# RandomMike1280/AlphaZero-Reversi

Measured on AMD Instinct MI355X. Metric: self-play board-steps/sec @ 800 sims/move, 8x8 Reversi, higher is better.
Workload: dtype u64 rules + f32 NN (fp32 as 2-part f16 split on MFMA)

## Files before the change

alphazero-reversi_amd/csrc/rvz_engine.hip:

```cpp
#include <hip/hip_bf16.h>
#include <hip/hip_runtime.h>
#include <math.h>
#include <stdint.h>
#include <stdio.h>
#include <stdlib.h>
#include <string.h>

#include <string>
#include <vector>

#include "../../include/rvz.h"
#include "rvz_h2.hip.h"
#include "rvz_pow.hip.h"
#include "rvz_rules.hip.h"
#include "rvz_trace.h"

using namespace rvz;

namespace {

constexpr int WAVE = 64;
constexpr int WPB = 4;
constexpr int PATH_CAP = 64;
constexpr int RNG_DRAWS = 64;
// ... 293 lines not shown
    if (copies == 0) return;
    const int path_reg = lane < plen ? v.path[g * PATH_CAP + lane] : 0;
    Node* nodes = v.nodes + (size_t)g * v.M;
    if (lane < plen) nodes[path_reg].n += copies;
    if (lane == 0) v.pend[g] = 0;
    __builtin_amdgcn_fence(__ATOMIC_SEQ_CST, "workgroup");
    if (v.stats) ab += 8ull + 4ull * plen + 8ull * plen;
}

template <int BS>
__device__ __forceinline__ int memo_expand_backup(const View& v, int g, int lane, int leaf,
                                                  uint32_t lm, int path_reg, int plen,
                                                  uint32_t lk, int copies,
                                                  unsigned long long& ab) {
    constexpr int NSQ = Geo<BS>::NSQ;
    Node* nodes = v.nodes + (size_t)g * v.M;
    uint32_t* meta = v.meta + (size_t)g * v.M;
    const int nch = link_nchild(lk), ob = 1 + link_block(lk) * NSQ;
    Node oc;
    uint32_t ocm = 0;
    if (lane < nch) {
        oc = nodes[ob + lane];
        ocm = meta[ob + lane];
    }
    const float val = v.bval[(size_t)g * 2 * v.E + link_block(lk)];
    const int e = v.nexp[g];
    const int base = 1 + e * NSQ;
    if (base + NSQ > v.M) {
        if (lane == 0) atomicOr(v.err, ERR_POOL);
        return -1;
    }
    float prior = lane < nch ? oc.p : 0.0f;
    if (leaf == 0 && v.noise_eps > 0.0f) {
        if (lane < nch) prior = root_noise_mix(v, g, m_sq(ocm), prior);
    }
    if (lane < nch) {
        Node c;
        c.n = 0; c.w = 0.0f; c.p = prior;
        const bool expd = m_nchild(ocm) > 0 && !m_term(ocm);
        c.c = __uint_as_float(expd ? link_pack(ob + lane, m_nchild(ocm), m_block(ocm))
                                   : LINK_NONE);
        nodes[base + lane] = c;
        meta[base + lane] = meta_pack(m_sq(ocm), 3 - m_turn(lm));
    }
    if (lane == 0) {
        meta[leaf] = lm | ((uint32_t)nch << 11) | ((uint32_t)e << 18);
        v.nexp[g] = e + 1;
        v.bval[(size_t)g * 2 * v.E + e] = val;
    }
    ab += 20ull * nch + 8 + 20ull * nch + 12 + 32ull * plen;
    return backup_path(nodes, path_reg, plen, val, copies, lane, true);
}

template <int BS, typename XT>
__device__ __forceinline__ int select_phase(const View& v, int g, int lane, int first, int bsz,
                                             int eb,
                                             const GameS& root, uint32_t root_meta, int root_n,
                                             uint32_t carry,
                                             XT* __restrict__ leaf_x, int32_t* __restrict__ need,
                                             unsigned long long& ab,
                                             uint64_t* leaf_bits = nullptr,
                                             bool unread = false) {
    constexpr int NSQ = Geo<BS>::NSQ;
    Node* nodes = v.nodes + (size_t)g * v.M;
    uint32_t* meta = v.meta + (size_t)g * v.M;
    if (first) {
        root_meta = meta_pack(0, root.side);
        root_n = 0;
        const int half = (v.memo && link_ok(carry) && (link_node(carry) - 1) / NSQ < v.E) ? 1 : 0;
        if (lane == 0) {
            Node r;
            r.n = 0; r.w = 0.0f; r.p = 1.0f; r.c = __int_as_float(0x7fc00000);
            nodes[0] = r;
            meta[0] = root_meta;
            v.nexp[g] = half * v.E;
        }
        const uint64_t rl = root.over ? 0ull : legal_wave<BS>(mine(root), theirs(root), lane);
        if (lane == 0) v.root_legal[g] = rl;
        if (v.noise_eps > 0.0f && rl != 0ull) root_noise_sample(v, g, lane, root, rl);
        ab += 20 + 8;
    }
    ab += 32 + 8;
    int copies = 0, plen = 0, path_reg = 0;
    if (!root.over) {
        int remaining = bsz;
        for (;;) {
            WALK_STAT(0, 1);
            WT_NOW(tw0);
            GameS sim = root;
            int depth = 0, node = 0, parent_n = root_n;
            uint32_t m = root_meta;
            uint32_t lk = first ? carry : LINK_NONE;
            path_reg = 0;
            int fp_ci = 0, fp_b = -1, fp_turn = 0;
            float fp_sb = 0.0f;
            bool truncated = false;
            int fp_sq = 0;
            for (;;) {
                const int nch = m_nchild(m);
                if (m_term(m) || nch == 0) break;
                const int base = 1 + m_block(m) * NSQ;
                Node c;
                uint32_t cm = 0;
                if (lane < nch) {
                    c = nodes[base + lane];
                    cm = meta[base + lane];
                } else {
                    c.n = 0; c.w = 0.0f; c.p = 0.0f; c.c = 0.0f;
                }
                float score = 0.0f;
                bool wrote = false;
                if (lane < nch) {
                    if (c.n == 0) {
                        score = INFINITY;
                    } else if (!isnan(c.c)) {
                        score = c.c;
                    } else {
                        const float sq_np = sqrt_count(parent_n);
                        score = ucb_score(c, sq_np, 3 - m_turn(m), v.cpuct);
                        nodes[base + lane].c = score;
                        wrote = true;
                    }
                }
                WALK_STAT(1, 1);
                const int ci = wave_argmax_first(score, lane < nch, lane);
                const int bsib = wave_argmax_first(score, lane < nch && lane != ci, lane);
                const float sbs = lane_bcast(score, bsib);
                const int turn_c = 3 - m_turn(m);
                if (v.stats) ab += 16ull * nch + 4ull * nch + 4ull * __popcll(__ballot(wrote));
                node = base + ci;
                m = (uint32_t)lane_bcast((int)cm, ci);
// ... 1405 lines not shown
    {
        double frac = e->gate_frac, us = e->gate_us, late = e->gate_late_us;
        if (frac < 0.0) {
            frac = RVZ_PLAY_GATE_FRAC;
            us = RVZ_PLAY_GATE_US;
            late = RVZ_PLAY_GATE_LATE_US;
        }
        if (const char* gs = getenv("RVZ_PLAY_GATE")) {
            double f = 0.0, u = 0.0, l = 0.0;
            const int n = sscanf(gs, "%lf,%lf,%lf", &f, &u, &l);
            frac = n >= 2 ? f : 0.0;
            us = u;
            late = n >= 3 ? l : 0.0;
        }
        pa.gate_frac = (queue && frac > 0.0 && us > 0.0)
                           ? (unsigned)(fmin(frac, 1.0) * 65536.0 + 0.5) : 0u;
        pa.gate_t = (unsigned)(us * 100.0);
        pa.gate_late = late > 0.0 ? (unsigned)(late * 100.0) : 0u;
    }
    sc += play_qwords(G);
    pa.x = sc;
    sc += play_al4(G * 3 * e->NSQ);
    pa.need = reinterpret_cast<int32_t*>(sc);
    sc += play_al4(G);
    pa.work = sc;
    sc += play_al4(G * 192);
    pa.logits = sc;
    sc += play_al4(G * e->NPOL);
    pa.value = sc;
    pa.ovf = a->ovf;
    pa.gpw = queue ? -a->games_per_workgroup : a->games_per_workgroup;
    pa.plies = a->plies;
    pa.skip_last = a->skip_last_eval && e->cfg.num_simulations > e->cfg.batch_size ? 1 : 0;
    pa.reset = a->reset ? 1 : 0;
    pa.S = e->cfg.num_simulations;
    pa.B = e->cfg.batch_size;
    pa.temperature = a->temperature;
    pa.seeds = a->seeds;
    pa.stride = a->seed_stride;
    pa.ply_ctr = a->plies_done;
    pa.done = a->games_done;
    pa.out_idx = a->out_idx;
    pa.out_p = a->out_p;
    pa.hist = a->hist;
    pa.rows = reinterpret_cast<unsigned long long*>(a->rows_evaluated);
    pa.budget = a->ply_budget;
    pa.tab = nullptr;
    pa.tclaim = nullptr;
    pa.tgen = nullptr;
    pa.tmask = 0;
    pa.tmaxd = 0;
    pa.tstats = reinterpret_cast<unsigned long long*>(a->table_stats);
    pa.unread = reinterpret_cast<unsigned long long*>(a->rows_unread);
    pa.rec_black = a->rec_black;
    pa.rec_white = a->rec_white;
    pa.rec_side = a->rec_side;
    pa.rec_p = a->rec_p;
    if ((a->rec_black || a->rec_white || a->rec_side || a->rec_p) &&
        !(a->rec_black && a->rec_white && a->rec_side && a->rec_p)) {
        e->err = "rvz_play: rec_black, rec_white, rec_side and rec_p go together";
        return RVZ_EINVAL;
    }
    if (e->tab) {
        if (e->tab_blob != a->blob) {
            if (e->tab_blob) {
                hipStreamCaptureStatus cs = hipStreamCaptureStatusNone;
                if (hipStreamIsCapturing(e->stream, &cs) == hipSuccess &&
                    cs != hipStreamCaptureStatusNone) {
                    e->err = "rvz_play: another weight blob than the table's while the stream is "
                             "capturing (play once eagerly with this evaluator before capturing)";
                    return RVZ_EINVAL;
                }
                const int r = table_bump(e);
                if (r != RVZ_OK) return r;
            }
            e->tab_blob = a->blob;
        }
        pa.tab = e->tab;
        pa.tclaim = e->tclaim;
        pa.tgen = e->tgen;
        pa.tmask = (unsigned)(e->tslots - 1);
        pa.tmaxd = e->tmaxd;
    }
    pa.spin_limit = 1u << 26;
    if (const char* sl = getenv("RVZ_PLAY_SPIN_LIMIT")) pa.spin_limit = (unsigned)strtoul(sl, nullptr, 10);
    e->searching = 0;
    if (e->BS == 8)
        return a->filters == 64    ? play_launch<64, 2, 2, 4, 8, 2>(e, v, pa, 2)
               : a->filters == 128 ? play_launch<128, 1, 2, 4, 8, 2>(e, v, pa, 2)
                                   : play_launch<256, 1, 4, 4, 8, 1>(e, v, pa, 1);
    return a->filters == 64 ? play_launch<64, 3, 2, 4, 6, 2>(e, v, pa, 2)
                            : play_launch<128, 1, 2, 3, 6, 2>(e, v, pa, 2);
}

struct rvz_timer {
    std::vector<hipEvent_t> ev;
};

int rvz_timer_create(int32_t n, rvz_timer** out) {
    if (n <= 0 || !out) return RVZ_EINVAL;
    rvz_timer* t = new rvz_timer;
    t->ev.resize(n, nullptr);
    for (auto& e : t->ev) {
        if (hipEventCreateWithFlags(&e, hipEventDisableSystemFence) != hipSuccess) {
            for (auto& f : t->ev)
                if (f) (void)hipEventDestroy(f);
// ... 106 lines not shown
```

alphazero-reversi_amd/csrc/rvz_play.hip.h:

```cpp

struct PlayArgs {
    const float* prm;
    Layout L;
    const uint16_t* blob;
    int n_blocks;
    float* x;
    int32_t* need;
    float* work;
    float* logits;
    float* value;
    float* ovf;
    int gpw, plies, skip_last, reset, S, B;
    double temperature;
    int64_t* seeds;
    int64_t stride;
    int64_t* ply_ctr;
    int64_t* done;
    int32_t* out_idx;
    double* out_p;
    int32_t* hist;
    unsigned long long* rows;
    const int32_t* budget;
    unsigned spin_limit;
    unsigned long long* tab;
    unsigned* tclaim;
    const unsigned* tgen;
    unsigned tmask;
    int tmaxd;
    unsigned long long* tstats;
    unsigned long long* unread;
    uint64_t* rec_black;
    uint64_t* rec_white;
    int32_t* rec_side;
    double* rec_p;
    unsigned* q_next;
    unsigned* q_done;
    int n_groups;
    unsigned long long* gate;
    unsigned gate_frac;
    unsigned gate_t;
    unsigned gate_late;
};
constexpr int PLAY_GPW_MAX = 64;
template <int F, int BS>
__host__ __device__ constexpr bool play_heads_lds() { return F == 64 && BS == 8; }
template <int F, int BS>
__host__ __device__ constexpr int play_gpw_max() {
    return play_heads_lds<F, BS>() ? 8 : PLAY_GPW_MAX;
}
enum : int { PF_QUEUED = 1, PF_READY = 2, PF_DONE = 4, PF_EVAL = 8, PF_HELD = 16 };
constexpr int32_t ERR_SCHED = 16;

template <int BS>
struct TabGeo {
    static constexpr int NSQ = Geo<BS>::NSQ;
    static constexpr int NG = NSQ + 8;
    static constexpr int STRIDE = (NG + 7) / 8 * 8;
};
constexpr int TAB_PROBES = 8;

__device__ __forceinline__ uint64_t tab_mix(uint64_t z) {
    z ^= z >> 30;
    z *= 0xbf58476d1ce4e5b9ull;
    z ^= z >> 27;
    z *= 0x94d049bb133111ebull;
    return z ^ (z >> 31);
}
__device__ __forceinline__ uint64_t tab_hash(uint64_t P, uint64_t O, uint64_t V) {
    return tab_mix(P ^ tab_mix(O ^ tab_mix(V + 0x9e3779b97f4a7c15ull)));
}
template <int NSQ>
__device__ __forceinline__ uint32_t tab_key_word(int idx, uint64_t P, uint64_t O, uint64_t V) {
    const int k = idx - (NSQ + 2);
    const uint64_t w = k < 2 ? P : (k < 4 ? O : V);
    return (k & 1) ? (uint32_t)(w >> 32) : (uint32_t)w;
}

template <int BS>
__device__ __forceinline__ int tab_read(const unsigned long long* __restrict__ tab, uint32_t sl,
                                         uint32_t gen, uint64_t P, uint64_t O, uint64_t V,
                                         int lane, uint64_t& x0, uint64_t& x1) {
    using T = TabGeo<BS>;
    constexpr int NSQ = T::NSQ, NG = T::NG;
    const unsigned long long* e = tab + (size_t)sl * T::STRIDE;
    x0 = 0;
    x1 = 0;
    if (lane < NG) x0 = __hip_atomic_load(e + lane, __ATOMIC_RELAXED, __HIP_MEMORY_SCOPE_AGENT);
    if (NG > 64 && lane < NG - 64)
        x1 = __hip_atomic_load(e + 64 + lane, __ATOMIC_RELAXED, __HIP_MEMORY_SCOPE_AGENT);
    bool stale = false, other = false;
    if (lane < NG) {
        stale |= (uint32_t)(x0 >> 32) != gen;
        if (lane >= NSQ + 2) other |= (uint32_t)x0 != tab_key_word<NSQ>(lane, P, O, V);
    }
// ... 145 lines not shown
    asm volatile("" : "+s"(p));
    return *(const PlayCtx*)p;
}

#ifdef RVZ_PLAY_TIMING
__device__ unsigned long long g_play_t[16384][12];
#define PT_NOW(t) const unsigned long long t = __builtin_amdgcn_s_memtime()
#define PT_ADD(i, v) if (tid == 0 && blockIdx.x < 16384) g_play_t[blockIdx.x][i] += (v)
#else
#define PT_NOW(t)
#define PT_ADD(i, v)
#endif

template <int F, int NBOARD, int CTW, int PTW, int BS, int OCC>
__global__ __launch_bounds__(256) __attribute__((amdgpu_waves_per_eu(OCC, OCC)))
void k_play(PlayCtx ctx0) {
    (void)ctx0;
    using WT = WaveTilesH<F, CTW, PTW>;
    constexpr bool ILV = RVZ_H2_ILV && NBOARD == 2 && BS == 8 && PTW == 4 && WT::CG == 2;
    using GH = GeoH<NBOARD, BS, 64 * CTW * H2_TM / F, ILV>;
    using C = CfgH<F, GH::NPIX>;
    constexpr int NPOL = Geo<BS>::NPOL;
    constexpr bool HLDS = play_heads_lds<F, BS>();
    constexpr int GMAX = play_gpw_max<F, BS>();
    constexpr int HROW = heads_in_floats(BS) / 16;
    constexpr int SP_BYTES = WPB * (NPOL + 7) * 8;
    static_assert(heads_in_floats(BS) * 4 <= C::RMAX, "heads rows fit");
    static_assert(SP_BYTES + WPB * 624 * 4 <= C::RMAX, "act / reset scratch fits");
    __shared__ __attribute__((aligned(16))) char smem[C::BYTES];
    __shared__ int st_k[GMAX];
    __shared__ int st_f[GMAX];
    __shared__ int st_p[GMAX];
    __shared__ uint64_t st_bits[GMAX * 3];
    __shared__ uint64_t q_bits[(GMAX + NBOARD) * 3];
    __shared__ __attribute__((aligned(16))) float hin[HLDS ? GMAX * HROW : 4];
    __shared__ int q_rows[GMAX + 16];
    __shared__ int s_nq;
    __shared__ float vpart[4][16];
    __shared__ int s_task[2];
    __shared__ unsigned s_tgen;
    const int tid = threadIdx.x;
    const int wave = __builtin_amdgcn_readfirstlane(tid >> 6);
    int E, G, gpw, total, queue, task_plies;
    {
        const PlayCtx& c = play_ctx();
        E = c.v.E;
        G = c.v.G;
        gpw = c.a.gpw;
        queue = c.a.q_next != nullptr;
        total = queue ? c.a.n_groups * c.a.plies : 0;
        task_plies = queue ? 1 : c.a.plies;
    }
    bool ovf = false;
    __shared__ unsigned s_cnt[4];
    if (tid < 4) s_cnt[tid] = 0u;
    if (tid == 0) {
        const PlayArgs& a = play_ctx().a;
        s_tgen = a.tab ? __hip_atomic_load(a.tgen, __ATOMIC_RELAXED, __HIP_MEMORY_SCOPE_AGENT) : 0u;
    }
    double* sp = reinterpret_cast<double*>(smem) + wave * (NPOL + 7);
    uint32_t* key = reinterpret_cast<uint32_t*>(smem + SP_BYTES) + wave * 624;
    if constexpr (F >= 128 && BS == 8) {
        const PlayArgs& a = play_ctx().a;
        if (tid == 0 && a.gate_frac > 0) gate_running(a.gate, 1);
    }
    PT_NOW(t_start);
    for (int task_i = 0;; ++task_i) {
        int gi, ply0;
        if (!queue) {
            if (task_i > 0) break;
            gi = blockIdx.x;
            ply0 = 0;
        } else {
            PT_NOW(t_q0);
            if (tid == 0) {
                const PlayCtx& c = play_ctx();
                const PlayArgs& a = c.a;
                const bool failed = __hip_atomic_load(c.v.err, __ATOMIC_RELAXED,
                                                      __HIP_MEMORY_SCOPE_AGENT) & ERR_SCHED;
                const unsigned t =
                    failed ? (unsigned)total
                           : __hip_atomic_fetch_add(a.q_next, 1u, __ATOMIC_RELAXED,
                                                    __HIP_MEMORY_SCOPE_AGENT);
                int tg = -1, tp = 0;
                if ((int)t < total) {
                    tg = (int)(t % (unsigned)a.n_groups);
                    tp = (int)(t / (unsigned)a.n_groups);
                    unsigned spins = 0;
                    while ((int)__hip_atomic_load(a.q_done + tg, __ATOMIC_RELAXED,
                                                  __HIP_MEMORY_SCOPE_AGENT) < tp) {
                        __builtin_amdgcn_s_sleep(4);
                        ++spins;
                        if (spins > a.spin_limit ||
                            ((spins & 1023u) == 0 &&
                             (__hip_atomic_load(c.v.err, __ATOMIC_RELAXED,
                                                __HIP_MEMORY_SCOPE_AGENT) & ERR_SCHED))) {
                            atomicOr(c.v.err, ERR_SCHED);
                            tg = -1;
                            break;
                        }
                    }
                    __builtin_amdgcn_fence(__ATOMIC_ACQUIRE, "agent");
                    asm volatile("s_waitcnt vmcnt(0)" ::: "memory");
                }
                s_task[0] = tg;
                s_task[1] = tp;
            }
            __syncthreads();
// ... 3 lines not shown
            PT_NOW(t_q1);
            PT_ADD(8, t_q1 - t_q0);
            PT_ADD(9, 1);
        }
        const int g0 = gi * gpw;
        const int ng = min(gpw, G - g0);
        {
            const int32_t* bud = play_ctx().a.budget;
            for (int j = tid; j < ng; j += 256) {
                st_k[j] = 0;
                st_f[j] = (bud && ply0 >= bud[g0 + j]) ? PF_DONE : 0;
                st_p[j] = 0;
            }
        }
        __syncthreads();
        for (;;) {
            PT_NOW(t_c0);
            for (int j = wave; j < ng; j += WPB) {
                const PlayCtx& c = play_ctx();
                const View& v = c.v;
                const PlayArgs& a = c.a;
                const int lane = opaque_tid() & 63;
                const int g = g0 + j;
                int f = __builtin_amdgcn_readfirstlane(st_f[j]);
                if (f & (PF_QUEUED | PF_DONE)) continue;
                int k = __builtin_amdgcn_readfirstlane(st_k[j]);
                int np = __builtin_amdgcn_readfirstlane(st_p[j]);
                WT_NOW(ft_step);
                FT_CNT();
                for (;;) {
                    unsigned long long ab = 0;
                    if (k < E) {
                        const int first = k == 0;
                        const GameS root = load_game(v, g);
                        uint32_t root_meta = 0, carry = LINK_NONE;
                        int root_n = 0;
                        if (!first) {
                            root_meta = v.meta[(size_t)g * v.M];
                            root_n = v.nodes[(size_t)g * v.M].n;
                        } else if (v.memo) {
                            carry = v.carry[g];
                        }
                        if (f & PF_READY) {
                            WT_NOW(ft_e);
                            const ExpIn x = expand_load<BS>(v, g, lane, a.logits, a.value);
                            const int rn =
                                expand_backup_phase<BS>(v, g, lane, x, 1, &root_meta, ab);
                            if (rn >= 0) root_n = rn;
                            f &= ~PF_READY;
                            FT_ADD(0, ft_e);
                        }
                        const int bsz = min(a.B, a.S - k * a.B);
                        const bool unread = a.skip_last && !first && m_nchild(root_meta) >= E - 1;
                        const int copies = select_phase<BS, float>(v, g, lane, first, bsz, k, root,
                                                                   root_meta, root_n, carry, a.x,
                                                                   a.need, ab, st_bits + 3 * j,
                                                                   unread);
                        ++k;
                        if (copies < 0 && k < E && lane == 0) atomicAdd(&s_cnt[3], 1u);
                        if (copies > 0 && !(k == E && a.skip_last)) {
                            if (a.tab) {
                                const uint64_t P = st_bits[3 * j], O = st_bits[3 * j + 1],
                                               Vb = st_bits[3 * j + 2];
                                WT_NOW(ft_t);
                                const bool hit = __popcll(P | O) <= a.tmaxd &&
                                                 tab_lookup<BS>(a, s_tgen, P, O, Vb, lane, g);
                                WT_ADD(0, ft_t);
                                if (hit) {
                                    __builtin_amdgcn_fence(__ATOMIC_SEQ_CST, "workgroup");
                                    f |= PF_READY;
                                    if (lane == 0) atomicAdd(&s_cnt[1], 1u);
                                    continue;
                                }
                            }
                            f |= PF_QUEUED;
                            break;
                        }
                        continue;
                    }
                    WT_NOW(ft_a);
                    bool over = false;
                    double* outp = a.out_p;
                    if (a.rec_black) {
                        const size_t ri = (size_t)(ply0 + np) * v.G + g;
                        if (lane == 0) {
                            a.rec_black[ri] = v.black[g];
                            a.rec_white[ri] = v.white[g];
                            a.rec_side[ri] = v.status[(size_t)g * 4];
                        }
                        outp = a.rec_p + (size_t)(ply0 + np) * v.G * Geo<BS>::NPOL;
                    }
                    const int idx = act_game<BS>(v, g, lane, sp, (f & PF_READY) ? 1 : 2,
                                                 a.logits, 1, a.value, a.temperature, nullptr, 1,
                                                 a.out_idx, outp, &over);
                    f &= ~PF_READY;
                    int64_t sd = 0;
                    if (lane == 0) {
                        if (idx >= 0) a.ply_ctr[g] += 1;
                        if (a.hist) a.hist[(size_t)(ply0 + np) * v.G + g] = idx;
                        if (a.reset && over) {
                            a.done[g] += 1;
                            sd = a.seeds[g] + a.stride;
                            a.seeds[g] = sd;
                        }
                    }
                    if (a.reset && over) {
                        sd = __shfl(sd, 0);
                        reset_game<BS>(v, g, lane, (uint32_t)(sd & 0xFFFFFFFFll), key);
                    }
                    FT_ADD(1, ft_a);
// ... 94 lines not shown
                    const PlayArgs& a = play_ctx().a;
                    const uint64_t P = q_bits[3 * i], O = q_bits[3 * i + 1], Vb = q_bits[3 * i + 2];
                    if (__popcll(P | O) <= a.tmaxd)
                        if (tab_insert<BS>(a, s_tgen, P, O, Vb, opaque_tid() & 63, q_rows[i]) &&
                            (opaque_tid() & 63) == 0)
                            atomicAdd(&s_cnt[2], 1u);
                }
            }
            for (int j = tid; j < ng; j += 256)
                if (st_f[j] & PF_EVAL) st_f[j] = (st_f[j] & ~(PF_QUEUED | PF_EVAL)) | PF_READY;
            __syncthreads();
            PT_NOW(t_c4);
            PT_ADD(2, t_c4 - t_c3);
        }
        if (queue) {
            asm volatile("s_waitcnt vmcnt(0)" ::: "memory");
            __syncthreads();
            if (tid == 0) {
                __builtin_amdgcn_fence(__ATOMIC_RELEASE, "agent");
                asm volatile("s_waitcnt vmcnt(0)" ::: "memory");
                __hip_atomic_store(play_ctx().a.q_done + gi, (unsigned)(ply0 + 1), __ATOMIC_RELAXED,
                                   __HIP_MEMORY_SCOPE_AGENT);
            }
        }
    }
    if constexpr (F >= 128 && BS == 8) {
        const PlayArgs& a = play_ctx().a;
        if (tid == 0 && a.gate_frac > 0) gate_running(a.gate, -1);
    }
#ifdef RVZ_PLAY_TIMING
    {
        PT_NOW(t_end);
        PT_ADD(3, t_end - t_start);
        if (tid == 0 && blockIdx.x < 16384)
            g_play_t[blockIdx.x][10] = __builtin_amdgcn_s_memrealtime();
        if (tid == 0 && blockIdx.x < 16384)
            g_play_t[blockIdx.x][7] =
                ((unsigned long long)__builtin_amdgcn_s_getreg((31 << 11) | 20) << 32) |
                __builtin_amdgcn_s_getreg((31 << 11) | 4);
    }
#endif
    float* ovw = play_ctx().a.ovf;
    if (ovf && ovw) *ovw = 1.0f;
    unsigned long long* rows = play_ctx().a.rows;
    __syncthreads();
    if (rows && tid == 0) atomicAdd(rows, (unsigned long long)s_cnt[0]);
    unsigned long long* ts = play_ctx().a.tstats;
    if (ts && tid == 0) {
        if (s_cnt[1]) atomicAdd(ts, (unsigned long long)s_cnt[1]);
        if (s_cnt[2]) atomicAdd(ts + 1, (unsigned long long)s_cnt[2]);
    }
    unsigned long long* un = play_ctx().a.unread;
    if (un && tid == 0 && s_cnt[3]) atomicAdd(un, (unsigned long long)s_cnt[3]);
}
```

alphazero-reversi_amd/rvz/_lib.py:

```python
from __future__ import annotations

import ctypes as C
import math
import numbers
import os

import torch

_HERE = os.path.dirname(os.path.abspath(__file__))
LIB_PATH = os.environ.get("RVZ_LIB", os.path.join(_HERE, "librvz.so"))

RVZ_OK, RVZ_DONE = 0, 1
RVZ_LEAF_F32, RVZ_LEAF_BF16 = 0, 1
RVZ_DRAWS = 64
RVZ_SOLVE_MAX_EMPTIES = 14
RVZ_SOLVE_NOT_A_MOVE, RVZ_SOLVE_ABANDONED = -128, -127


class RvzError(RuntimeError):
    pass


class Config(C.Structure):
    _fields_ = [("board_size", C.c_int32), ("n_games", C.c_int32),
# ... 42 lines not shown
    "rvz_search_rows_total": (C.c_int, [_P, C.POINTER(C.c_int64)]),
    "rvz_timer_create": (C.c_int, [C.c_int32, C.POINTER(C.c_void_p)]),
    "rvz_timer_record": (C.c_int, [_P, C.c_int32, _P]),
    "rvz_timer_elapsed": (C.c_int, [_P, C.c_int32, C.c_int32, C.POINTER(C.c_float)]),
    "rvz_timer_destroy": (None, [_P]),
    "rvz_search_skip": (C.c_int, [_P]),
    "rvz_search_visits": (C.c_int, [_P, _P]),
    "rvz_act": (C.c_int, [_P, C.c_double, _P, C.c_int32, _P, _P]),
    "rvz_act_schedule": (C.c_int, [_P, C.c_int32, C.c_double]),
    "rvz_action_probs": (C.c_int, [C.c_int32, C.c_int32, _P, _P, _P, _P, _P, _P, _P]),
    "rvz_solve": (C.c_int, [C.c_int32, C.c_int32, _P, _P, _P, C.c_int32, C.c_int64, _P, _P, _P,
                            _P]),
    "rvz_solve_window": (C.c_int, [C.c_int32, C.c_int32, _P, _P, _P, C.c_int32, C.c_int64,
                                   C.c_int32, C.c_int32, C.c_int32, _P, _P, _P, _P]),
    "rvz_solve_moves": (C.c_int, [C.c_int32, C.c_int32, _P, _P, _P, C.c_int32, C.c_int64,
                                  C.c_int32, C.c_int32, C.c_int32, _P, _P, _P, _P]),
    "rvz_play_scratch_size": (C.c_int64, [_P]),
    "rvz_play": (C.c_int, [_P, _P]),
    "rvz_play_table": (C.c_int, [_P, C.c_int64, C.c_int32]),
    "rvz_play_gate": (C.c_int, [_P, C.c_double, C.c_double, C.c_double]),
    "rvz_counters": (C.c_int, [_P, C.POINTER(C.c_int64)]),
    "rvz_stats_enable": (C.c_int, [_P, C.c_int32]),
    "rvz_stats_read": (C.c_int, [_P, C.POINTER(C.c_int64)]),
    "rvz_timing_enable": (C.c_int, [_P, C.c_int32]),
    "rvz_timing_read": (C.c_int, [_P, C.POINTER(C.c_double), C.POINTER(C.c_int32)]),
    "rvz_tree_nodes": (C.c_int, [_P]),
    "rvz_tree_export": (C.c_int, [_P, _P, _P]),
    "rvz_footprint": (C.c_int, [_P, C.POINTER(C.c_int64), C.POINTER(C.c_int64)]),
    "rvz_resnet_params_size": (C.c_int64, [C.c_int32, C.c_int32, C.c_int32]),
    "rvz_resnet_work_size": (C.c_int64, [C.c_int32]),
    "rvz_resnet_heads_fc": (C.c_int, [C.c_int32, _P, C.c_int32, _P, C.c_int32, C.c_int32, _P, _P,
                                      _P]),
    "rvz_resnet_h2_size": (C.c_int64, [C.c_int32, C.c_int32]),
    "rvz_resnet_h2_weights": (C.c_int, [_P, C.c_int32, C.c_int32, _P, _P]),
    "rvz_resnet_trunk_h2": (C.c_int, [C.c_int32, _P, C.c_int32, _P, _P, C.c_int32, C.c_int32,
                                      _P, _P]),
    "rvz_resnet_fwd_h2": (C.c_int, [C.c_int32, _P, C.c_int32, _P, _P, C.c_int32, C.c_int32, _P,
                                    _P, _P, _P]),
}

_lib = None


class PlayArgs(C.Structure):
    _fields_ = [("params", C.c_void_p), ("blob", C.c_void_p), ("filters", C.c_int32),
                ("blocks", C.c_int32), ("scratch", C.c_void_p), ("ovf", C.c_void_p),
                ("plies", C.c_int32), ("skip_last_eval", C.c_int32), ("reset", C.c_int32),
                ("games_per_workgroup", C.c_int32), ("temperature", C.c_double),
                ("seeds", C.c_void_p), ("seed_stride", C.c_int64), ("plies_done", C.c_void_p),
                ("games_done", C.c_void_p), ("out_idx", C.c_void_p), ("out_p", C.c_void_p),
                ("hist", C.c_void_p), ("rows_evaluated", C.c_void_p),
                ("ply_budget", C.c_void_p), ("table_stats", C.c_void_p),
                ("rec_black", C.c_void_p), ("rec_white", C.c_void_p), ("rec_side", C.c_void_p),
                ("rec_p", C.c_void_p), ("rows_unread", C.c_void_p)]


def load() -> C.CDLL:
    global _lib
    if _lib is None:
        if not os.path.exists(LIB_PATH):
            raise RvzError(f"{LIB_PATH} is missing: build it with `make -C alphazero-reversi_amd` "
                           "(there is no CPU fallback for the rvz hot path)")
        lib = C.CDLL(LIB_PATH, mode=C.RTLD_GLOBAL)
        for name, (res, args) in SIGNATURES.items():
            fn = getattr(lib, name)
            fn.restype = res
            fn.argtypes = args
        _lib = lib
    return _lib


_NO_EPSILON = object()


def check_noise_args(alpha, epsilon=_NO_EPSILON) -> None:
    try:
        a = float(alpha)
    except (TypeError, ValueError, OverflowError):
        raise RvzError(f"root noise: alpha must be a positive finite number, not {alpha!r}")
    if not 1.0e-37 <= a <= 3.0e38:
        raise RvzError(f"root noise: alpha must be positive and finite (float32), not {alpha!r}")
    if epsilon is not _NO_EPSILON:
        try:
            e = float(epsilon)
        except (TypeError, ValueError):
            raise RvzError(f"root noise: epsilon must be a number in [0, 1], not {epsilon!r}")
        if not 0.0 <= e <= 1.0:
            raise RvzError(f"root noise: epsilon must be in [0, 1], not {epsilon!r}")


def check_schedule_args(moves, late_temperature=0.0):
    if moves is None:
        return None
    if isinstance(moves, bool) or not isinstance(moves, numbers.Integral) or moves < 0:
        raise RvzError(f"temperature schedule: moves must be None or an int >= 0, not {moves!r}")
    if int(moves) > 2 ** 31 - 5:
        raise RvzError(f"temperature schedule: moves = {moves!r} is out of range")
    try:
        late = float(late_temperature)
    except (TypeError, ValueError, OverflowError):
        raise RvzError("temperature schedule: late_temperature must be a finite number >= 0, "
                       f"not {late_temperature!r}")
    if isinstance(late_temperature, bool) or not (0.0 <= late < math.inf):
        raise RvzError("temperature schedule: late_temperature must be a finite number >= 0, "
                       f"not {late_temperature!r}")
    return int(moves), late

# ... 54 lines not shown
```

alphazero-reversi_amd/rvz/engine.py:

```python
from __future__ import annotations

import ctypes as C
from typing import Callable, Optional, Sequence, Tuple

import torch

from . import _lib
from ._lib import RVZ_DONE, RVZ_LEAF_BF16, RVZ_LEAF_F32, RvzError, check, ptr

U64 = 0xFFFFFFFFFFFFFFFF
SOLVE_MAX_EMPTIES = _lib.RVZ_SOLVE_MAX_EMPTIES
SOLVE_NOT_A_MOVE = _lib.RVZ_SOLVE_NOT_A_MOVE
SOLVE_ABANDONED = _lib.RVZ_SOLVE_ABANDONED


def to_signed64(x: int) -> int:
    x &= U64
    return x - (1 << 64) if x >> 63 else x


def to_unsigned64(x: int) -> int:
    return int(x) & U64


# ... 162 lines not shown
        torch.cuda.current_stream(self.device).synchronize()

    def _env_snapshot(self):
        self._stream()
        b = torch.empty(self.n_games, dtype=torch.int64, device=self.device)
        w = torch.empty_like(b)
        st = torch.empty(self.n_games, 4, dtype=torch.int32, device=self.device)
        self._call("rvz_env_get", ptr(b), ptr(w), ptr(st))
        return b, w, st

    def solve(self, max_empties: int = SOLVE_MAX_EMPTIES, node_limit: int = 2 ** 24):
        b, w, st = self._env_snapshot()
        return solve(b, w, st, self.board_size, max_empties, node_limit)

    def solve_wld(self, max_empties: int = SOLVE_MAX_EMPTIES, node_limit: int = 2 ** 24,
                  order_min_empties: Optional[int] = None):
        b, w, st = self._env_snapshot()
        if order_min_empties is None:
            order_min_empties = WLD_ORDER_MIN_EMPTIES
        return solve_wld(b, w, st, self.board_size, max_empties, node_limit, order_min_empties)

    def solve_moves(self, max_empties: int = SOLVE_MAX_EMPTIES, node_limit: int = 2 ** 24,
                    alpha: int = -64, beta: int = 64, order_min_empties: int = 0):
        b, w, st = self._env_snapshot()
        return solve_moves(b, w, st, self.board_size, max_empties, node_limit, alpha, beta,
                           order_min_empties)

    def solve_moves_wld(self, max_empties: int = SOLVE_MAX_EMPTIES, node_limit: int = 2 ** 24,
                        order_min_empties: Optional[int] = None):
        b, w, st = self._env_snapshot()
        if order_min_empties is None:
            order_min_empties = WLD_ORDER_MIN_EMPTIES
        return solve_moves_wld(b, w, st, self.board_size, max_empties, node_limit,
                               order_min_empties)

    def legal(self) -> torch.Tensor:
        self._stream()
        out = torch.empty(self.n_games, dtype=torch.int64, device=self.device)
        self._call("rvz_env_legal", ptr(out))
        return out

    def apply(self, sq: torch.Tensor) -> torch.Tensor:
        self._stream()
        s = sq.to(self.device, torch.int32).contiguous()
        ok = torch.empty(self.n_games, dtype=torch.int32, device=self.device)
        self._call("rvz_env_apply", ptr(s), ptr(ok))
        return ok

    def play_buffers(self, evaluator=None):
        if getattr(self, "play_rows", None) is None:
            self.play_rows = torch.zeros(1, dtype=torch.int64, device=self.device)
            self.table_stats = torch.zeros(2, dtype=torch.int64, device=self.device)
            self.play_unread = torch.zeros(1, dtype=torch.int64, device=self.device)
        n = self.lib.rvz_play_scratch_size(self._h)
        sc = getattr(self, "_play_scratch", None)
        if sc is None or sc.numel() < n:
            self._play_scratch = torch.zeros(n, dtype=torch.float32, device=self.device)
        if evaluator is not None and hasattr(evaluator, "ovf_word"):
            evaluator.ovf_word()

    def play(self, evaluator, plies: int, temperature: float, seeds: torch.Tensor, stride: int,
             plies_done: torch.Tensor, games_done: torch.Tensor, reset: bool = True,
             skip_last_eval: bool = False, hist: Optional[torch.Tensor] = None,
             games_per_workgroup: int = 0, budget: Optional[torch.Tensor] = None,
             records=None):
        from .network import LeafEvaluator
        if not isinstance(evaluator, LeafEvaluator):
            raise RvzError("play() runs the h2 LeafEvaluator inside the launch; another "
                           "evaluator goes through search() / act()")
        if evaluator.board_size != self.board_size or evaluator.device != self.device:
            raise RvzError("play(): the evaluator's board size / device differ from the engine's")
        for t, dt in ((seeds, torch.int64), (plies_done, torch.int64), (games_done, torch.int64)):
            if t.dtype != dt or t.numel() != self.n_games or not t.is_contiguous():
                raise RvzError("play: seeds / plies_done / games_done int64 [n_games]")
        if hist is not None and (hist.dtype != torch.int32 or hist.shape != (plies, self.n_games)
                                 or not hist.is_contiguous()):
            raise RvzError("play: hist int32 [plies, n_games]")
        if budget is not None and (budget.dtype != torch.int32 or budget.numel() != self.n_games
                                   or not budget.is_contiguous()
                                   or budget.device != self.device):
            raise RvzError("play: budget int32 [n_games] on the engine's device")
        rec = (None,) * 4
        if records is not None and hist is None:
            raise RvzError("play: records need hist (the moves of the recorded plies)")
        if records is not None:
            rb, rw, rs, rp = records
            G = self.n_games
            if not (rb.dtype == rw.dtype == torch.int64 and rs.dtype == torch.int32
                    and rp.dtype == torch.float64 and rb.shape == rw.shape == rs.shape
                    == (plies, G) and rp.shape == (plies, G, self.npol)
                    and all(t.is_contiguous() and t.device == self.device
                            for t in (rb, rw, rs, rp))):
                raise RvzError("play: records = (black int64, white int64 [plies, G], side int32 "
                               "[plies, G], p float64 [plies, G, npol]) on the engine's device")
            rec = tuple(t.data_ptr() for t in records)
        n = self.lib.rvz_play_scratch_size(self._h)
        ready = (getattr(self, "play_rows", None) is not None and
                 getattr(self, "_play_scratch", None) is not None and
                 self._play_scratch.numel() >= n and getattr(evaluator, "_ovf", None) is not None)
        if not ready:
            if torch.cuda.is_current_stream_capturing():
                raise RvzError("play() inside a graph capture before its buffers exist: call "
                               "Engine.play_buffers(evaluator) (or one eager play) first")
            self.play_buffers(evaluator)
        sc = self._play_scratch
        self._bind(evaluator)
        a = _lib.PlayArgs(evaluator.params.data_ptr(), evaluator.wsplit.data_ptr(),
                          evaluator.filters, evaluator.n_blocks, sc.data_ptr(),
                          evaluator.ovf_word().data_ptr(), int(plies), int(bool(skip_last_eval)),
                          int(bool(reset)), int(games_per_workgroup), float(temperature),
                          seeds.data_ptr(), int(stride), plies_done.data_ptr(),
                          games_done.data_ptr(), self.idx_buf.data_ptr(), self.p_buf.data_ptr(),
                          hist.data_ptr() if hist is not None else None,
                          self.play_rows.data_ptr(),
                          budget.data_ptr() if budget is not None else None,
                          self.table_stats.data_ptr(), *rec, self.play_unread.data_ptr())
        self._stream()
        self._call("rvz_play", C.byref(a))

    def _bind(self, evaluator):
        evs = self.__dict__.setdefault("_evaluators", [])
        if not any(e is evaluator for e in evs):
            evs.append(evaluator)
            reg = getattr(evaluator, "bind_engine", None)
            if reg is not None:
                reg(self)

    def table(self, slots: int = 1 << 20, max_discs: int = 14):
        self._stream()
        self._call("rvz_play_table", int(slots), int(max_discs))
        self.table_slots = int(slots)

    def play_gate(self, fraction: float = -1.0, timeout_us: float = 0.0, late_us: float = 0.0):
        self._call("rvz_play_gate", float(fraction), float(timeout_us), float(late_us))

    def root_noise(self, alpha: float, epsilon: float, salt: int = 0):
        _lib.check_noise_args(alpha, epsilon)
        self._call("rvz_search_root_noise", float(alpha), float(epsilon), int(salt) & 0xFFFFFFFF)
        self.noise = (float(alpha), float(epsilon), int(salt) & 0xFFFFFFFF)

    def temperature_schedule(self, moves: Optional[int], late_temperature: float = 0.0):
        sched = _lib.check_schedule_args(moves, late_temperature)
        if sched is None:
            self._call("rvz_act_schedule", 0, 0.0)
        else:
            self._call("rvz_act_schedule", 4 + sched[0], sched[1])
        self.schedule = sched

    def search_begin(self):
        self._call("rvz_search_begin")

    def search_step(self) -> bool:
        self._stream()
        rc = self._call("rvz_search_step", ptr(self.leaf_x), ptr(self.need))
        return rc != RVZ_DONE

    def compact(self, on: bool = True):
        self._call("rvz_search_compact", int(bool(on)))
        self.compact_leaves = bool(on)

    def memo(self, on: bool = True):
        self._stream()
        self._call("rvz_search_memo", int(bool(on)))
        self.memo_on = bool(on)

    def memo_reset(self):
        self._stream()
        self._call("rvz_search_memo_reset")

# ... 232 lines not shown
```

alphazero-reversi_amd/rvz/selfplay.py:

```python
from __future__ import annotations

import os
import time
from datetime import datetime
from typing import Callable, Dict, List, Optional, Sequence

import numpy as np
import torch

from .engine import Engine, board_canonical


class SelfPlayRunner:
    def __init__(self, engine: Engine, evaluator: Callable, temperature: float = 1.0,
                 fused_softmax: bool = True, autoreset: bool = False, seed_base: int = 42,
                 record: bool = False, max_plies: int = 60, seed_stride: int = None,
                 skip_last_eval: bool = False, fused_bookkeeping: bool = True,
                 fused: bool = False, temperature_schedule=None):
        self.eng = engine
        if temperature_schedule is not None:
            engine.temperature_schedule(*temperature_schedule)
        self.skip_last_eval = bool(skip_last_eval)
        self.fused = bool(fused)
        self.play_group = 0
        if self.fused and not fused_softmax:
            raise ValueError("the fused runner plays with fused_softmax")
        if self.fused and record and autoreset:
            raise ValueError("a recording fused runner plays whole games (no autoreset)")
        self.fused_bookkeeping = bool(fused_bookkeeping)
        self.evaluator = evaluator
        self.temperature = float(temperature)
        self.fused_softmax = fused_softmax
        self.autoreset = autoreset
        self.seed_base = seed_base
        self.seed_stride = engine.n_games if seed_stride is None else int(seed_stride)
        self.record = record
        G, dev = engine.n_games, engine.device
        self.seeds = (torch.arange(G, dtype=torch.int64, device=dev) + seed_base)
        self._plies = torch.zeros(G, dtype=torch.int64, device=dev)
        self._done = torch.zeros(G, dtype=torch.int64, device=dev)
        self.pre_black = torch.zeros(G, dtype=torch.int64, device=dev)
        self.pre_white = torch.zeros(G, dtype=torch.int64, device=dev)
        self.pre_status = torch.zeros(G, 4, dtype=torch.int32, device=dev)
        self.post_status = torch.zeros(G, 4, dtype=torch.int32, device=dev)
        self._seed32 = torch.zeros(G, dtype=torch.int32, device=dev)
        self._mask = torch.zeros(G, dtype=torch.uint8, device=dev)
        self.graph: Optional[torch.cuda.CUDAGraph] = None
        if record:
            self.rec_black = torch.zeros(max_plies, G, dtype=torch.int64, device=dev)
            self.rec_white = torch.zeros(max_plies, G, dtype=torch.int64, device=dev)
            self.rec_side = torch.zeros(max_plies, G, dtype=torch.int32, device=dev)
            self.rec_idx = torch.full((max_plies, G), -2, dtype=torch.int32, device=dev)
            self.rec_p = torch.zeros(max_plies, G, engine.npol, dtype=torch.float64, device=dev)
            self.rec_over = torch.zeros(max_plies, G, 4, dtype=torch.int32, device=dev)
        self.ply_index = 0
        if self.fused:
            engine.play_buffers(evaluator)

    @property
    def steps(self) -> torch.Tensor:
        return self._plies.sum()

    @property
    def games_done(self) -> torch.Tensor:
        return self._done.sum()

    def start(self):
        self.eng.reset(self.seeds)
        self.ply_index = 0

    def check(self):
        self.eng.check()

    def _body(self, plies: int = 1):
        eng = self.eng
        if self.fused:
            rec, hist = None, None
            if self.record:
                k, n = self.ply_index, plies
                if k + n > self.rec_idx.shape[0]:
                    raise ValueError("records are full (max_plies)")
                rec = (self.rec_black[k:k + n], self.rec_white[k:k + n], self.rec_side[k:k + n],
                       self.rec_p[k:k + n])
                hist = self.rec_idx[k:k + n]
            eng.play(self.evaluator, plies, self.temperature, self.seeds, self.seed_stride,
                     self._plies, self._done, reset=self.autoreset,
                     skip_last_eval=self.skip_last_eval, hist=hist,
                     games_per_workgroup=self.play_group, records=rec)
            if self.record:
                self.post_status.copy_(eng.get_state()[2])
            return
        if self.record:
            b, w, st = eng.get_state()
            self.pre_black.copy_(b)
            self.pre_white.copy_(w)
            self.pre_status.copy_(st)
        eng.search(self.evaluator, fused_softmax=self.fused_softmax,
                   skip_last_eval=self.skip_last_eval)
        idx, _ = eng.act(self.temperature, apply=True)
        if self.record:
            self.post_status.copy_(eng.get_state()[2])
        if self.fused_bookkeeping:
            eng.autoreset(idx, self.seeds, self.seed_stride, self._plies, self._done,
                          reset=self.autoreset)
            return
        self._plies += (idx >= 0).to(torch.int64)
        if self.autoreset:
            self.restart_finished(eng.get_state()[2])

    def restart_finished(self, status: torch.Tensor):
        over = status[:, 1]
        self._done += over.to(torch.int64)
        self.seeds += over.to(torch.int64) * self.seed_stride
        self._mask.copy_(over.to(torch.uint8))
        self._seed32.copy_(self.seeds.bitwise_and(0xFFFFFFFF).to(torch.int32))
        self.eng.reset_device(self._seed32, self._mask)

    def capture(self, plies: int = 1):
        if plies < 1 or (plies > 1 and self.record and not self.fused) or (self.record and
                                                                          self.fused):
            raise ValueError("plies >= 1; a recording runner captures one ply per graph (the "
                             "fused recording runner writes to the ply's record slice: use "
                             "play_record)")
        torch.cuda.synchronize(self.eng.device)
        g = torch.cuda.CUDAGraph()
        with torch.cuda.graph(g):
            if self.fused:
                self._body(plies)
            else:
                for _ in range(plies):
                    self._body()
        self.graph = g
        self.plies_per_call = int(plies)
        torch.cuda.synchronize(self.eng.device)

    plies_per_call = 1

    def play_record(self, plies: int):
        if not (self.fused and self.record):
            raise ValueError("play_record is the fused recording runner's")
        self._body(plies)
# ... 319 lines not shown
```

include/rvz.h:

```cpp
#ifndef RVZ_H
#define RVZ_H
#include <stdint.h>

#ifdef __cplusplus
extern "C" {
#endif

#define RVZ_OK 0
#define RVZ_DONE 1
#define RVZ_EINVAL (-22)
#define RVZ_ENOMEM (-12)
#define RVZ_EHIP (-5)
#define RVZ_EDEVICE (-71)

#define RVZ_LEAF_F32 0
#define RVZ_LEAF_BF16 1

#define RVZ_LIVE_STRIPE 128
#define RVZ_LIVE_PITCH 16

typedef struct rvz_engine rvz_engine;

typedef struct rvz_config {
    int32_t board_size;
// ... 48 lines not shown
                        const uint32_t *seed32, const int32_t *tag, uint32_t salt, double alpha,
                        float *out, uint32_t *out_bits, void *hip_stream);
int rvz_search_rows_total(rvz_engine *e, int64_t *out );
int rvz_search_visits(rvz_engine *e, int32_t *out);
int rvz_act(rvz_engine *e, double temperature, const double *u, int32_t apply, int32_t *out_idx,
            double *out_p);
int rvz_act_schedule(rvz_engine *e, int32_t from_discs, double late_temperature);
int rvz_action_probs(int32_t board_size, int32_t n, const int32_t *visits,
                     const double *temperature, const double *u, int32_t *out_idx, double *out_p,
                     int32_t *out_drew, void *hip_stream);

#define RVZ_SOLVE_MAX_EMPTIES 14
int rvz_solve(int32_t board_size, int32_t n, const uint64_t *black, const uint64_t *white,
              const int32_t *status, int32_t max_empties, int64_t node_limit, int32_t *out_score,
              int32_t *out_move, int64_t *out_nodes, void *hip_stream);
int rvz_solve_window(int32_t board_size, int32_t n, const uint64_t *black, const uint64_t *white,
                     const int32_t *status, int32_t max_empties, int64_t node_limit,
                     int32_t alpha, int32_t beta, int32_t order_min_empties,
                     int32_t *out_score, int32_t *out_move, int64_t *out_nodes, void *hip_stream);
#define RVZ_SOLVE_NOT_A_MOVE (-128)
#define RVZ_SOLVE_ABANDONED (-127)
int rvz_solve_moves(int32_t board_size, int32_t n, const uint64_t *black, const uint64_t *white,
                    const int32_t *status, int32_t max_empties, int64_t node_limit,
                    int32_t alpha, int32_t beta, int32_t order_min_empties, int32_t *out_scores,
                    int32_t *out_count, int64_t *out_nodes, void *hip_stream);

typedef struct rvz_play_args {
    const float *params;
    const uint16_t *blob;
    int32_t filters;
    int32_t blocks;
    float *scratch;
    float *ovf;
    int32_t plies;
    int32_t skip_last_eval;
    int32_t reset;
    int32_t games_per_workgroup;
    double temperature;
    int64_t *seeds;
    int64_t seed_stride;
    int64_t *plies_done;
    int64_t *games_done;
    int32_t *out_idx;
    double *out_p;
    int32_t *hist;
    int64_t *rows_evaluated;
    const int32_t *ply_budget;
    int64_t *table_stats;
    uint64_t *rec_black;
    uint64_t *rec_white;
    int32_t *rec_side;
    double *rec_p;
    int64_t *rows_unread;
} rvz_play_args;
int64_t rvz_play_scratch_size(const rvz_engine *e);
int rvz_play(rvz_engine *e, const rvz_play_args *a);
int rvz_play_table(rvz_engine *e, int64_t slots, int32_t max_discs);
int rvz_play_gate(rvz_engine *e, double fraction, double timeout_us, double late_us);

typedef struct rvz_timer rvz_timer;
int rvz_timer_create(int32_t n_events, rvz_timer **out);
int rvz_timer_record(rvz_timer *t, int32_t i, void *hip_stream);
int rvz_timer_elapsed(rvz_timer *t, int32_t i, int32_t j, float *ms );
void rvz_timer_destroy(rvz_timer *t);

int rvz_counters(const rvz_engine *e, int64_t *out2 );
int rvz_stats_enable(rvz_engine *e, int32_t on);
int rvz_stats_read(rvz_engine *e, int64_t *out3 );
int rvz_timing_enable(rvz_engine *e, int32_t on);
int rvz_timing_read(rvz_engine *e, double *out_ms , int32_t *out_n );
int rvz_tree_nodes(const rvz_engine *e);
int rvz_tree_export(rvz_engine *e, void *nodes_out, uint32_t *meta_out);
int rvz_footprint(const rvz_engine *e, int64_t *bytes_tree, int64_t *bytes_env);

int64_t rvz_resnet_params_size(int32_t board, int32_t filters, int32_t blocks);
int64_t rvz_resnet_work_size(int32_t n);
int rvz_resnet_heads_fc(int32_t board, const float *work, int32_t n, const float *params,
                        int32_t filters, int32_t blocks, float *logits, float *value,
                        void *hip_stream);

int64_t rvz_resnet_h2_size(int32_t filters, int32_t blocks);
int rvz_resnet_h2_weights(const float *params, int32_t filters, int32_t blocks, uint16_t *blob,
                          void *hip_stream);
int rvz_resnet_fwd_h2(int32_t board, const float *x, int32_t n, const float *params,
                      const uint16_t *blob, int32_t filters, int32_t blocks, float *work,
                      float *logits, float *value, void *hip_stream);
int rvz_resnet_trunk_h2(int32_t board, const float *x, int32_t n, const float *params,
                        const uint16_t *blob, int32_t filters, int32_t blocks, float *work,
                        void *hip_stream);
int32_t rvz_resnet_h2_grid(int32_t board, int32_t filters, int32_t n);
int rvz_resnet_fwd_h2_ex(int32_t board, const float *x, int32_t n, const float *params,
                         const uint16_t *blob, int32_t filters, int32_t blocks, float *work,
                         float *logits, float *value, const int32_t *n_live, void *hip_stream);
int rvz_resnet_trunk_h2_ex(int32_t board, const float *x, int32_t n, const float *params,
                           const uint16_t *blob, int32_t filters, int32_t blocks, float *work,
                           const int32_t *n_live, uint64_t *stamps, const uint32_t *stamp_ctr,
                           int32_t ring, void *hip_stream);
int rvz_resnet_heads_fc_ex(int32_t board, const float *work, int32_t n, const float *params,
                           int32_t filters, int32_t blocks, float *logits, float *value,
                           const int32_t *n_live, uint32_t *stamp_ctr, void *hip_stream);

#ifdef __cplusplus
}
#endif
#endif
```

Measured before the change: 1.666 million.

## Short-circuit root search when legal moves cover all batches

When a fresh root has at least E-1 legal moves and skip_last_eval is on, a new forced_search routine builds the root's children directly. It gives them deterministic visit counts, reuses subtrees linked from the previous move, and returns early, skipping the per-batch select/evaluate loop. The point is to avoid NN leaf evaluations and tree walks whose outcome the batch schedule already fixes. Risks: it assumes the search would spread visits across distinct children, and it writes zero priors with unevaluated children. It is enabled by default only for fused play with skip_last_eval and at least 3 batches, and adds a roots_unread counter.

Result: faster. 1.711 million, median of 6 (+2.7%).

```diff
diff --git a/alphazero-reversi_amd/csrc/rvz_engine.hip b/alphazero-reversi_amd/csrc/rvz_engine.hip
--- a/alphazero-reversi_amd/csrc/rvz_engine.hip
+++ b/alphazero-reversi_amd/csrc/rvz_engine.hip
@@ -369,6 +369,81 @@
     return backup_path(nodes, path_reg, plen, val, copies, lane, true);
 }
 
+struct Forced {
+    int E, S, B;
+};
+
+template <int BS>
+__device__ __noinline__ int forced_search(const View& v, int g, int lane, int side,
+                                          uint32_t root_meta, uint64_t rl, int half,
+                                          uint32_t carry, Forced fz) {
+    constexpr int NSQ = Geo<BS>::NSQ;
+    Node* nodes = v.nodes + (size_t)g * v.M;
+    uint32_t* meta = v.meta + (size_t)g * v.M;
+    const int L = __popcll(rl), nv = fz.E - 1;
+    const int e0 = half * v.E, base = 1 + e0 * NSQ;
+    const bool linked_root = v.memo && link_ok(carry);
+    const bool mine = lane < NSQ && ((rl >> lane) & 1ull);
+    const int idx = __popcll(rl & ((1ull << lane) - 1ull));
+    if (base + NSQ > v.M) {
+        if (lane == 0) atomicOr(v.err, ERR_POOL);
+        return 0;
+    }
+    uint32_t lk = LINK_NONE;
+    if (linked_root && mine) {
+        const int oc = 1 + link_block(carry) * NSQ + idx;
+        const uint32_t ocm = meta[oc];
+        if (m_nchild(ocm) > 0 && !m_term(ocm)) lk = link_pack(oc, m_nchild(ocm), m_block(ocm));
+    }
+    const bool visited = mine && idx < nv;
+    uint64_t lmask = __ballot(visited && link_ok(lk));
+    if (1 + (e0 + 1 + __popcll(lmask)) * NSQ > v.M) {
+        if (lane == 0) atomicOr(v.err, ERR_POOL);
+        lmask = 0ull;
+    }
+    const bool expd = (lmask >> lane) & 1ull;
+    const int ce = e0 + 1 + __popcll(lmask & ((1ull << lane) - 1ull));
+    if (mine) {
+        Node c;
+        c.n = visited ? min(fz.B, fz.S - (idx + 1) * fz.B) : 0;
+        c.w = 0.0f; c.p = 0.0f; c.c = __uint_as_float(LINK_NONE);
+        nodes[base + idx] = c;
+        uint32_t cm = meta_pack(lane, 3 - side);
+        if (expd) cm |= ((uint32_t)link_nchild(lk) << 11) | ((uint32_t)ce << 18);
+        meta[base + idx] = cm;
+    }
+    int e = e0 + 1;
+    for (uint64_t rest = lmask; rest != 0ull; rest &= rest - 1ull, ++e) {
+        const int s = __ffsll((unsigned long long)rest) - 1;
+        const uint32_t l = (uint32_t)__builtin_amdgcn_readlane((int)lk, s);
+        const int nch = link_nchild(l), ob = 1 + link_block(l) * NSQ, nb = 1 + e * NSQ;
+        if (lane < nch) {
+            const Node oc = nodes[ob + lane];
+            const uint32_t ocm = meta[ob + lane];
+            Node c;
+            c.n = 0; c.w = 0.0f; c.p = oc.p;
+            c.c = __uint_as_float(m_nchild(ocm) > 0 && !m_term(ocm)
+                                      ? link_pack(ob + lane, m_nchild(ocm), m_block(ocm))
+                                      : LINK_NONE);
+            nodes[nb + lane] = c;
+            meta[nb + lane] = meta_pack(m_sq(ocm), side);
+        }
+        if (lane == 0)
+            v.bval[(size_t)g * 2 * v.E + e] = v.bval[(size_t)g * 2 * v.E + link_block(l)];
+    }
+    if (lane == 0) {
+        Node r;
+        r.n = fz.S; r.w = 0.0f; r.p = 1.0f; r.c = __int_as_float(0x7fc00000);
+        nodes[0] = r;
+        meta[0] = root_meta | ((uint32_t)L << 11) | ((uint32_t)e0 << 18);
+        v.nexp[g] = e;
+        v.pend[g] = 0;
+        v.plen[g] = 0;
+    }
+    __builtin_amdgcn_fence(__ATOMIC_SEQ_CST, "workgroup");
+    return __popcll(__ballot(mine && idx < nv - 1 && !link_ok(lk))) + (linked_root ? 0 : 256);
+}
+
 template <int BS, typename XT>
 __device__ __forceinline__ int select_phase(const View& v, int g, int lane, int first, int bsz,
                                              int eb,
@@ -377,7 +452,7 @@
                                              XT* __restrict__ leaf_x, int32_t* __restrict__ need,
                                              unsigned long long& ab,
                                              uint64_t* leaf_bits = nullptr,
-                                             bool unread = false) {
+                                             bool unread = false, Forced fz = Forced{0, 0, 0}) {
     constexpr int NSQ = Geo<BS>::NSQ;
     Node* nodes = v.nodes + (size_t)g * v.M;
     uint32_t* meta = v.meta + (size_t)g * v.M;
@@ -394,6 +469,8 @@
         }
         const uint64_t rl = root.over ? 0ull : legal_wave<BS>(mine(root), theirs(root), lane);
         if (lane == 0) v.root_legal[g] = rl;
+        if (fz.E > 0 && !root.over && __popcll(rl) >= fz.E - 1)
+            return -2 - forced_search<BS>(v, g, lane, root.side, root_meta, rl, half, carry, fz);
         if (v.noise_eps > 0.0f && rl != 0ull) root_noise_sample(v, g, lane, root, rl);
         ab += 20 + 8;
     }
@@ -1905,6 +1982,8 @@
     pa.tmaxd = 0;
     pa.tstats = reinterpret_cast<unsigned long long*>(a->table_stats);
     pa.unread = reinterpret_cast<unsigned long long*>(a->rows_unread);
+    pa.skip_forced = a->skip_forced_roots && pa.skip_last ? 1 : 0;
+    pa.roots_unread = reinterpret_cast<unsigned long long*>(a->roots_unread);
     pa.rec_black = a->rec_black;
     pa.rec_white = a->rec_white;
     pa.rec_side = a->rec_side;
diff --git a/alphazero-reversi_amd/csrc/rvz_play.hip.h b/alphazero-reversi_amd/csrc/rvz_play.hip.h
--- a/alphazero-reversi_amd/csrc/rvz_play.hip.h
+++ b/alphazero-reversi_amd/csrc/rvz_play.hip.h
@@ -40,6 +40,8 @@
     unsigned gate_frac;
     unsigned gate_t;
     unsigned gate_late;
+    int skip_forced;
+    unsigned long long* roots_unread;
 };
 constexpr int PLAY_GPW_MAX = 64;
 template <int F, int BS>
@@ -291,8 +293,8 @@
         task_plies = queue ? 1 : c.a.plies;
     }
     bool ovf = false;
-    __shared__ unsigned s_cnt[4];
-    if (tid < 4) s_cnt[tid] = 0u;
+    __shared__ unsigned s_cnt[5];
+    if (tid < 5) s_cnt[tid] = 0u;
     if (tid == 0) {
         const PlayArgs& a = play_ctx().a;
         s_tgen = a.tab ? __hip_atomic_load(a.tgen, __ATOMIC_RELAXED, __HIP_MEMORY_SCOPE_AGENT) : 0u;
@@ -402,10 +404,20 @@
                         }
                         const int bsz = min(a.B, a.S - k * a.B);
                         const bool unread = a.skip_last && !first && m_nchild(root_meta) >= E - 1;
+                        const Forced fz{first && a.skip_forced ? E : 0, a.S, a.B};
                         const int copies = select_phase<BS, float>(v, g, lane, first, bsz, k, root,
                                                                    root_meta, root_n, carry, a.x,
                                                                    a.need, ab, st_bits + 3 * j,
-                                                                   unread);
+                                                                   unread, fz);
+                        if (copies <= -2) {
+                            k = E;
+                            const int left = -2 - copies;
+                            if (lane == 0) {
+                                if (left & 255) atomicAdd(&s_cnt[3], (unsigned)(left & 255));
+                                if (left >> 8) atomicAdd(&s_cnt[4], 1u);
+                            }
+                            continue;
+                        }
                         ++k;
                         if (copies < 0 && k < E && lane == 0) atomicAdd(&s_cnt[3], 1u);
                         if (copies > 0 && !(k == E && a.skip_last)) {
@@ -606,4 +618,6 @@
     }
     unsigned long long* un = play_ctx().a.unread;
     if (un && tid == 0 && s_cnt[3]) atomicAdd(un, (unsigned long long)s_cnt[3]);
-}
+    unsigned long long* ur = play_ctx().a.roots_unread;
+    if (ur && tid == 0 && s_cnt[4]) atomicAdd(ur, (unsigned long long)s_cnt[4]);
+}
diff --git a/alphazero-reversi_amd/rvz/_lib.py b/alphazero-reversi_amd/rvz/_lib.py
--- a/alphazero-reversi_amd/rvz/_lib.py
+++ b/alphazero-reversi_amd/rvz/_lib.py
@@ -118,7 +118,8 @@
                 ("hist", C.c_void_p), ("rows_evaluated", C.c_void_p),
                 ("ply_budget", C.c_void_p), ("table_stats", C.c_void_p),
                 ("rec_black", C.c_void_p), ("rec_white", C.c_void_p), ("rec_side", C.c_void_p),
-                ("rec_p", C.c_void_p), ("rows_unread", C.c_void_p)]
+                ("rec_p", C.c_void_p), ("rows_unread", C.c_void_p),
+                ("skip_forced_roots", C.c_int32), ("roots_unread", C.c_void_p)]
 
 
 def load() -> C.CDLL:
diff --git a/alphazero-reversi_amd/rvz/engine.py b/alphazero-reversi_amd/rvz/engine.py
--- a/alphazero-reversi_amd/rvz/engine.py
+++ b/alphazero-reversi_amd/rvz/engine.py
@@ -238,6 +238,8 @@
             self.play_rows = torch.zeros(1, dtype=torch.int64, device=self.device)
             self.table_stats = torch.zeros(2, dtype=torch.int64, device=self.device)
             self.play_unread = torch.zeros(1, dtype=torch.int64, device=self.device)
+        if getattr(self, "play_roots_unread", None) is None:
+            self.play_roots_unread = torch.zeros(1, dtype=torch.int64, device=self.device)
         n = self.lib.rvz_play_scratch_size(self._h)
         sc = getattr(self, "_play_scratch", None)
         if sc is None or sc.numel() < n:
@@ -249,7 +251,7 @@
              plies_done: torch.Tensor, games_done: torch.Tensor, reset: bool = True,
              skip_last_eval: bool = False, hist: Optional[torch.Tensor] = None,
              games_per_workgroup: int = 0, budget: Optional[torch.Tensor] = None,
-             records=None):
+             records=None, skip_forced_roots: bool = False):
         from .network import LeafEvaluator
         if not isinstance(evaluator, LeafEvaluator):
             raise RvzError("play() runs the h2 LeafEvaluator inside the launch; another "
@@ -282,6 +284,7 @@
             rec = tuple(t.data_ptr() for t in records)
         n = self.lib.rvz_play_scratch_size(self._h)
         ready = (getattr(self, "play_rows", None) is not None and
+                 getattr(self, "play_roots_unread", None) is not None and
                  getattr(self, "_play_scratch", None) is not None and
                  self._play_scratch.numel() >= n and getattr(evaluator, "_ovf", None) is not None)
         if not ready:
@@ -300,7 +303,8 @@
                           hist.data_ptr() if hist is not None else None,
                           self.play_rows.data_ptr(),
                           budget.data_ptr() if budget is not None else None,
-                          self.table_stats.data_ptr(), *rec, self.play_unread.data_ptr())
+                          self.table_stats.data_ptr(), *rec, self.play_unread.data_ptr(),
+                          int(bool(skip_forced_roots)), self.play_roots_unread.data_ptr())
         self._stream()
         self._call("rvz_play", C.byref(a))
 
diff --git a/alphazero-reversi_amd/rvz/selfplay.py b/alphazero-reversi_amd/rvz/selfplay.py
--- a/alphazero-reversi_amd/rvz/selfplay.py
+++ b/alphazero-reversi_amd/rvz/selfplay.py
@@ -16,11 +16,13 @@
                  fused_softmax: bool = True, autoreset: bool = False, seed_base: int = 42,
                  record: bool = False, max_plies: int = 60, seed_stride: int = None,
                  skip_last_eval: bool = False, fused_bookkeeping: bool = True,
-                 fused: bool = False, temperature_schedule=None):
+                 fused: bool = False, temperature_schedule=None, skip_forced_roots=None):
         self.eng = engine
         if temperature_schedule is not None:
             engine.temperature_schedule(*temperature_schedule)
         self.skip_last_eval = bool(skip_last_eval)
+        self.skip_forced_roots = (bool(fused) and bool(skip_last_eval) and engine.n_batches >= 3
+                                  if skip_forced_roots is None else bool(skip_forced_roots))
         self.fused = bool(fused)
         self.play_group = 0
         if self.fused and not fused_softmax:
@@ -86,7 +88,8 @@
             eng.play(self.evaluator, plies, self.temperature, self.seeds, self.seed_stride,
                      self._plies, self._done, reset=self.autoreset,
                      skip_last_eval=self.skip_last_eval, hist=hist,
-                     games_per_workgroup=self.play_group, records=rec)
+                     games_per_workgroup=self.play_group, records=rec,
+                     skip_forced_roots=self.skip_forced_roots)
             if self.record:
                 self.post_status.copy_(eng.get_state()[2])
             return
diff --git a/include/rvz.h b/include/rvz.h
--- a/include/rvz.h
+++ b/include/rvz.h
@@ -124,6 +124,8 @@
     int32_t *rec_side;
     double *rec_p;
     int64_t *rows_unread;
+    int32_t skip_forced_roots;
+    int64_t *roots_unread;
 } rvz_play_args;
 int64_t rvz_play_scratch_size(const rvz_engine *e);
 int rvz_play(rvz_engine *e, const rvz_play_args *a);
```
